# apache/orc

Measured on AMD Instinct MI355X. Metric: decoded GB/s + Mvalues/s device-resident, RLEv2 int64 column at 1/2/4/8 GPU, higher is better.
Workload: dtype int64; 1 GPU; configs[1]: single int64 RLEv2-direct column, 10^8 rows, uncompressed stream resident in HBM, 1 MI355X per stripe; rows_per_gpu=100000000, encoding=RLEv2 DIRECT, W=64 (aligned), 512-value runs, signed (zigzag), stream_bytes=800390626, row_index_stride=10000, parallelism=stripe-sharded x1, kernel=rlev2_tiled_kernel, variant=0

## Files before the change

orc_amd/csrc/orcg_internal.hh:

```
#pragma once

#include <hip/hip_runtime.h>
#include <stdint.h>

#include <algorithm>
#include <string>
#include <vector>

#include "../../include/orcg.h"

namespace orcg {

enum DevErr : uint32_t {
  kErrNone = 0,
  kErrBadRead = 1,
  kErrPatchedPl0 = 2,
  kErrPatchedWidth = 3,
  kErrDeltaLength = 4,
  kErrBadSegment = 5,
  kErrByteBadRead = 6,
  kErrDictIndex = 7,
  kErrV1BadRead = 8,
  kErrDecimalScale = 9,
  kErrHive11Overflow = 10,
// ... 26 lines not shown
  uint64_t lb_cap = 0;
  uint32_t lb_epoch = 0;
  void* d_rtab = nullptr;
  uint64_t rtab_cap = 0;
  void* d_rhdr = nullptr;
  uint64_t rhdr_cap = 0;
  void* h_jobs = nullptr;
  void* d_jobs = nullptr;
  uint64_t jobs_cap = 0, jobs_used = 0;
  uint8_t* arena_h = nullptr;
  uint8_t* arena_d = nullptr;
  uint64_t arena_cap = 0, arena_used = 0;
  std::vector<Ctx*> lanes;
  hipEvent_t ev_fork = nullptr;
  std::vector<hipEvent_t> ev_join;
};

Ctx* ctx_lane(Ctx* base, size_t k);
void warm_rlev2_walk(hipStream_t s);
void warm_rlev2_tiled(hipStream_t s);
void warm_byterle(hipStream_t s);
void warm_columns(hipStream_t s);
void warm_rlev1(hipStream_t s);
void warm_decimal(hipStream_t s);

unsigned side_lanes();

struct RleJob {
  const uint8_t* src;
  uint64_t src_len;
  const uint64_t* segtab;
  const int64_t* trip;
  const int64_t* rows;
  uint64_t nsegs;
  void* dst;
  uint64_t nvalues;
  uint64_t seg_base;
  uint32_t is_signed;
  uint32_t tab_base;
  unsigned long long* err;
  const uint64_t* dcount;
};

struct V1SegDesc {
  const uint8_t* src;
  uint64_t src_len;
  uint64_t seg_start, vi;
  uint64_t seg_end, v_next;
  void* dst;
  uint64_t nvalues;
  unsigned long long* err;
  uint32_t is_signed, pad;
};

int set_error(Ctx* ctx, int status, const std::string& msg);
bool debug_on(const char* topic);
void debug_stale(const char* where);
void* pinned_alloc(size_t bytes, int node = -1);
int current_numa_node();
void pinned_free(void* p);
int hip_check(Ctx* ctx, hipError_t e, const char* what);
int scratch(Ctx* ctx, int slot, size_t bytes, void** out);
int sync_ctx(Ctx* ctx);

int launch_rlev2_decode(Ctx* ctx, const uint8_t* d_src, uint64_t src_len, int is_signed,
                        const uint64_t* d_segtab, uint64_t nsegs, bool positions_mode,
                        uint64_t rows_per_group, uint64_t value_begin, uint64_t nvalues,
                        void* d_dst, int dst_bytes, int java = 0);


constexpr uint32_t kRtHdr = 6;
constexpr uint32_t kSliceMax = 1024;
struct RunTab {
  uint64_t* tab;
  uint32_t* hdr;
  uint32_t spg;
  uint32_t slice;
};
int launch_rlev2_expand(Ctx* ctx, const uint8_t* d_src, uint64_t src_len, int is_signed, uint64_t value_begin,
                        uint64_t nvalues, void* d_dst, int dst_bytes, const uint64_t* d_count, const RleJob* jobs_d,
                        uint32_t njobs, uint64_t nsegs, const RunTab& rt);
void warm_rlev2_expand(hipStream_t s);

constexpr int kMaxRlev2Variant = 9;
bool rlev2_variant_valid(int v);
int launch_rlev2_tiled(Ctx* ctx, const uint8_t* d_src, uint64_t src_len, int is_signed,
                       const uint64_t* d_segtab, uint64_t nsegs, bool positions_mode,
                       uint64_t rows_per_group, uint64_t value_begin, uint64_t nvalues,
                       void* d_dst, int dst_bytes, const uint64_t* d_count = nullptr);

int launch_rlev2_multi(Ctx* ctx, const RleJob* jobs, uint32_t njobs);
bool rlev2_multi_capable(int variant);
int stage_table(Ctx* ctx, const void* src, size_t bytes, const void** out);
inline int stage_rle_jobs(Ctx* ctx, const RleJob* jobs, uint32_t n, const RleJob** out) {
  return stage_table(ctx, jobs, (size_t)n * sizeof(RleJob), (const void**)out);
}

struct MultiLaunch {
  int kind;
  int variant;
  const void* d_jobs;
  uint32_t njobs;
  uint64_t grid;
  uint64_t values;
  uint64_t tab_entries = 0;
  uint32_t spg = 0, slice = 0;
};
int plan_rlev2_multi(Ctx* ctx, const RleJob* jobs, uint32_t njobs, std::vector<MultiLaunch>& out);
struct VarintJob {
  const uint8_t* src;
  uint64_t len;
  int64_t* counts;
  int64_t* base;
  uint64_t* total;
};
struct ScanJob {
  const int64_t* in;
  uint64_t n;
  int64_t* out;
  uint64_t* flags;
  uint64_t* total;
};
int plan_rlev1_multi(Ctx* ctx, const V1SegDesc* segs, uint64_t nsegs, std::vector<MultiLaunch>& out);
int run_multi(Ctx* ctx, const std::vector<MultiLaunch>& launches);

int launch_byterle(Ctx* ctx, const uint8_t* d_src, uint64_t src_len, const uint64_t* d_segtab, uint64_t nsegs,
                   bool boolean, uint64_t begin, uint64_t nout, uint8_t* d_dst, uint64_t* d_ones = nullptr,
                   const uint64_t* d_nout = nullptr);
int launch_rlev1(Ctx* ctx, const uint8_t* d_src, uint64_t src_len, int is_signed, const uint64_t* d_segtab,
                 uint64_t nsegs, uint64_t value_begin, uint64_t nvalues, void* d_dst, int dst_bytes);
int launch_rlev1_multi(Ctx* ctx, const V1SegDesc* segs, uint64_t nsegs);
int launch_rlev1_jobs(Ctx* ctx, const V1SegDesc* d_segs, uint64_t nsegs, int chunk);
int launch_scatter(Ctx* ctx, const void* d_dense, const uint8_t* d_nn, uint64_t n, void* d_out, int width,
                   int fill_mode, int64_t fill);
int launch_dict_offsets(Ctx* ctx, const int64_t* d_lengths, uint64_t dict_size, int64_t* d_offsets,
                        uint64_t* d_summary = nullptr);
int launch_dict_gather(Ctx* ctx, const void* d_idx, int idx_width, const uint8_t* d_nn, uint64_t n,
                       const int64_t* d_offsets, uint64_t dict_size, int64_t* d_start, int64_t* d_len);
constexpr uint32_t kDictLds = 4096;
struct DictJob {
  const int64_t* lengths;
  uint64_t dict_size;
  int64_t* offsets;
  uint64_t* summary;
  const int64_t* idx;
  const uint8_t* nn;
  uint64_t n;
  int64_t* start;
  int64_t* len;
  unsigned long long* err;
  uint64_t tile_base;
};
int launch_dict_multi(Ctx* ctx, const DictJob* jobs, uint32_t njobs);
int plan_dict_multi(Ctx* ctx, const DictJob* jobs, uint32_t njobs, std::vector<MultiLaunch>& out);
int launch_dict_jobs(Ctx* ctx, const DictJob* d_jobs, uint32_t njobs, uint64_t tiles);

int launch_varint_tile_counts(Ctx* ctx, const uint8_t* d_src, uint64_t len, int64_t* d_counts, uint64_t* ntiles);
constexpr uint64_t kVarintTile = 4096;
int launch_varint_decimal(Ctx* ctx, const uint8_t* d_src, uint64_t len, const int64_t* d_tile_base,
                          const int64_t* d_scales, uint64_t nvalues, int32_t scale, int mode, void* d_out,
                          uint8_t* d_keep = nullptr);
struct DecJob {
  const uint8_t* src;
  uint64_t len;
  const int64_t* tile_base;
  const int64_t* scales;
  uint64_t nvalues;
// ... 67 lines not shown
```

orc_amd/csrc/rlev2_tiled.hip:

```cpp
#include <algorithm>
#include <cstring>
#include <type_traits>
#include <vector>

#include "rlev2_device.hh"

namespace orcg {
namespace {
using namespace dev;

#ifdef ORCG_PHASE_PROF
__device__ unsigned long long g_phase[16];
constexpr uint32_t kWgDurMax = 16384;
__device__ unsigned long long g_wgdur[2 * kWgDurMax];
#define PROF_MARK(k)                                                        \
  do {                                                                      \
    if (threadIdx.x == 0) {                                                 \
      const uint64_t now_ = wall_clock64();                                 \
      atomicAdd(&g_phase[k], (unsigned long long)(now_ - prof_last_));      \
      prof_last_ = now_;                                                    \
    }                                                                       \
  } while (0)
#define PROF_DECL uint64_t prof_last_ = wall_clock64()
#else
#define PROF_MARK(k) \
  do {               \
  } while (0)
#define PROF_DECL
#endif

constexpr int kThreads = 256;
constexpr int kWaves = kThreads / kWave;
constexpr uint32_t kMaxRun = 4608;

constexpr uint32_t kSlab = 2048;
constexpr uint32_t kBlk = kSlab / kThreads;
constexpr uint32_t kDenseRuns = kSlab / 2;
constexpr uint32_t kStage = 256;
constexpr uint32_t kShortL = 16;
constexpr uint32_t kVparL = 256;
#ifndef ORCG_VPAR_MIN
#define ORCG_VPAR_MIN 16
#endif
constexpr uint32_t kVparMin = ORCG_VPAR_MIN;
#ifndef ORCG_VPAR_FRAG
#define ORCG_VPAR_FRAG 2
#endif
constexpr uint32_t kVparFrag = ORCG_VPAR_FRAG;
#ifndef ORCG_FLAT_RUNS
#define ORCG_FLAT_RUNS 2
#endif
constexpr uint32_t kNone = 0xffffffffu;
constexpr uint32_t kDpErr = 0x80000000u;
constexpr uint16_t kSink = 0xffffu;
constexpr uint32_t kWalkDone = 0x80000000u;
constexpr uint32_t kToDense = 24, kToSerial = 64;
#ifndef ORCG_TAB_TO_DENSE
#define ORCG_TAB_TO_DENSE 128
#endif
#ifndef ORCG_TAB_TO_SERIAL
#define ORCG_TAB_TO_SERIAL 512
#endif
constexpr uint32_t kTabToDense = ORCG_TAB_TO_DENSE, kTabToSerial = ORCG_TAB_TO_SERIAL;

constexpr int kOptNTStore = 1;
constexpr int kOptNTLoad = 2;
constexpr int kOptReuse = 4;
constexpr int kOptFast = 8;
constexpr int kOptRegFill = 16;
constexpr int kOptT4 = 32;
constexpr int kOptD3 = 64;
constexpr int kOptDirect = 128;
constexpr int kOptPair = 256;
constexpr int kOptUnion = 1024;
constexpr int kOptScan = 4096;
constexpr int kOptPrefetch = 2048;
constexpr int kOptGrpT = 8192;
constexpr int kOptTable = 16384;
constexpr int kOptFlat = 32768;

#ifdef ORCG_DEBUG_COVER
#define ORCG_COVER_ADD(x) atomicAdd(s_cover_ptr(), (uint32_t)(x))
__device__ __forceinline__ uint32_t* s_cover_ptr() {
  __shared__ uint32_t s_cover;
  return &s_cover;
}
#else
#define ORCG_COVER_ADD(x) \
  do {                    \
  } while (0)
#endif

template <int kOpt, typename T>
__device__ __forceinline__ void store1(T* p, uint64_t v) {
  if constexpr ((kOpt & kOptNTStore) != 0) __builtin_nontemporal_store((T)(int64_t)v, p);
  else *p = (T)(int64_t)v;
}

typedef uint64_t u64x2 __attribute__((ext_vector_type(2)));
template <int kOpt>
__device__ __forceinline__ void store2(int64_t* p, uint64_t a, uint64_t b) {
  u64x2 v;
  v.x = a;
  v.y = b;
  if constexpr ((kOpt & kOptNTStore) != 0) __builtin_nontemporal_store(v, (u64x2*)p);
  else *(u64x2*)p = v;
}

__device__ __forceinline__ uint32_t lds_byte(const uint32_t* w, uint32_t o) {
  return (w[o >> 2] >> ((o & 3u) * 8)) & 0xffu;
}

__device__ __forceinline__ u32x3 lds12(const uint32_t* w, uint32_t o) {
  const uint32_t i = o >> 2;
  u32x3 r;
  r.x = w[i];
  r.y = w[i + 1];
  r.z = w[i + 2];
  return r;
}

constexpr uint32_t kHdrLim = 64;

__device__ __forceinline__ uint32_t term4(uint32_t w) {
  const uint32_t m = (~w >> 7) & 0x01010101u;
  return (m * 0x10204080u) >> 28;
}

struct LaneWin {
  uint32_t word = 0, base = 0xffffffffu;
  uint32_t t4 = 0;
  __device__ __forceinline__ void load(const uint32_t* win, uint32_t hoff, uint32_t nwords, int lane) {
    base = hoff & ~3u;
    uint32_t idx = (base >> 2) + (uint32_t)lane;
    if (idx >= nwords) idx = nwords - 1;
    word = win[idx];
    t4 = term4(word);
  }
  __device__ __forceinline__ void cover(const uint32_t* win, uint32_t hoff, uint32_t nwords, int lane) {
    if (base == 0xffffffffu || hoff < base || hoff + kHdrLim > base + 256) load(win, hoff, nwords, lane);
  }
  __device__ __forceinline__ uint32_t byte(uint32_t o) const {
    o -= base;
    return (rdlane(word, o >> 2) >> ((o & 3u) * 8)) & 0xffu;
  }
};

template <int kOpt, typename T>
__device__ __forceinline__ void expand_run(const uint32_t* win, uint32_t nwords, uint32_t hoff, uint64_t v0,
                                           int is_signed, uint64_t value_begin, uint64_t value_end, T* dst,
                                           int lane) {
  LaneWin hw;
  hw.load(win, hoff, nwords, lane);
  Run r;
  if ((hw.byte(hoff) >> 6) == 3) {
    const uint32_t fb = hw.byte(hoff);
    r.kind = 3;
    r.pbs = r.pl = r.cfb = 0;
    r.err = kErrNone;
    r.L = ((fb & 1u) << 8 | hw.byte(hoff + 1)) + 1u;
    const uint32_t fbo = (fb >> 1) & 0x1fu;
    r.W = fbo ? fbs_width(fbo) : 0u;
// ... 191 lines not shown
    for (int it = 0; it < kMaxRunUnroll; ++it) {
      const uint32_t j = it * kWave + lane;
      const uint64_t o = v0 + j;
      if ((uint32_t)it < niter && j < L && o >= value_begin && o < value_end)
        store1<kOpt>(dst + (o - value_begin), r.a + (uint64_t)j * r.b);
    }
    return;
  }
  const uint32_t W = r.W;
  const uint64_t v1 = r.a + r.b;
  const bool neg = (int64_t)r.b < 0;
  uint64_t carry = 0;
  if (W <= 26 && (kOpt & kOptFast) && L == 512 && v0 >= value_begin && v0 + 512 <= value_end) {
    T* out = dst + (v0 - value_begin);
    uint32_t dl[kMaxRunUnroll];
#pragma unroll
    for (int it = 0; it < kMaxRunUnroll; ++it) {
      const uint32_t j = it * kWave + lane;
      const uint32_t k = j >= 2 ? j - 2 : 0u;
      const uint32_t bit = k * W;
      const uint32_t br = d + (bit >> 3);
      dl[it] = (uint32_t)field(lds12(win, br), br, bit & 7u, W);
    }
    if (lane < 2) dl[0] = 0;
#pragma unroll
    for (int it = 0; it < kMaxRunUnroll; ++it) {
      const uint32_t j = it * kWave + lane;
      const uint32_t s32 = wave_scan_u32(dl[it]);
      const uint64_t sum = carry + s32;
      carry += (uint32_t)__builtin_amdgcn_readlane((int)s32, 63);
      const uint64_t v = j == 0 ? r.a : (j == 1 ? v1 : (neg ? v1 - sum : v1 + sum));
      store1<kOpt>(out + j, v);
    }
    return;
  }
  if (W <= 26) {
#pragma unroll 1
    for (uint32_t it = 0; it < niter; ++it) {
      const uint32_t j = it * kWave + lane;
      const int32_t k = (int32_t)j - 2;
      uint32_t dlt = 0;
      if (k >= 0 && j < L) {
        const uint32_t bit = (uint32_t)k * W;
        const uint32_t br = d + (bit >> 3);
        dlt = (uint32_t)field(lds12(win, br), br, bit & 7u, W);
      }
      const uint32_t s32 = wave_scan_u32(dlt);
      const uint64_t sum = carry + s32;
      carry += (uint32_t)__builtin_amdgcn_readlane((int)s32, 63);
      const uint64_t v = j == 0 ? r.a : (j == 1 ? v1 : (neg ? v1 - sum : v1 + sum));
      const uint64_t o = v0 + j;
      if (j < L && o >= value_begin && o < value_end) store1<kOpt>(dst + (o - value_begin), v);
    }
    return;
  }
#pragma unroll 1
  for (uint32_t it = 0; it < niter; ++it) {
    const uint32_t j = it * kWave + lane;
    const int32_t k = (int32_t)j - 2;
    uint64_t dlt = 0;
    if (k >= 0 && j < L) {
      const uint32_t bit = (uint32_t)k * W;
      const uint32_t br = d + (bit >> 3);
      dlt = field(lds12(win, br), br, bit & 7u, W);
    }
    const uint64_t sum = wave_inclusive_scan(dlt) + carry;
    carry = last_lane(sum);
    const uint64_t v = j == 0 ? r.a : (j == 1 ? v1 : (neg ? v1 - sum : v1 + sum));
    const uint64_t o = v0 + j;
    if (j < L && o >= value_begin && o < value_end) store1<kOpt>(dst + (o - value_begin), v);
  }
}

template <int kOpt>
__device__ __forceinline__ void fill(uint32_t* win, __amdgpu_buffer_rsrc_t rs, uint32_t wrel,
                                     uint32_t bytes, int w, int nw, int lane) {
  for (uint32_t off = w * 1024u; off < bytes; off += nw * 1024u)
    __builtin_amdgcn_raw_ptr_buffer_load_lds(rs, (__attribute__((address_space(3))) void*)((char*)win + off),
                                             16, wrel + off + lane * 16, 0, 0,
                                             (kOpt & kOptNTLoad) ? 2 : 0);
}

__device__ __forceinline__ uint32_t flat_probe(__amdgpu_buffer_rsrc_t rs, uint32_t prel, uint32_t lim,
                                               uint32_t kmax, int lane, uint32_t* nb) {
  uint32_t h[4];
#pragma unroll
  for (uint32_t wi = 0; wi < 4; ++wi) {
    const uint32_t B = 2u + 512u * (5u + wi);
    const uint64_t off = (uint64_t)prel + (uint32_t)lane * B;
    uint32_t x = 0;
    if ((uint32_t)lane < kmax && off + B <= lim) {
      const auto q = __builtin_amdgcn_raw_buffer_load_b64(rs, (uint32_t)off & ~3u, 0, 0);
      const uint64_t qq = ((uint64_t)q[1] << 32) | q[0];
      x = (uint32_t)(qq >> (((uint32_t)off & 3u) * 8u)) & 0xffffu;
    }
    h[wi] = x;
  }
  const uint32_t hdr = uni(h[0]);
  if ((hdr & 0xfff9u) != 0xff79u) return 0;
  const uint32_t wi = (hdr >> 1) & 3u;
  const uint32_t mine = wi == 0 ? h[0] : (wi == 1 ? h[1] : (wi == 2 ? h[2] : h[3]));
  const uint64_t differ = ~__ballot(mine == hdr);
  *nb = 5u + wi;
  return differ ? (uint32_t)__builtin_ctzll(differ) : 64u;
}

template <int kOpt, int kRuns, typename T>
__device__ __forceinline__ void flat_expand(__amdgpu_buffer_rsrc_t rs, uint32_t d, uint32_t dstep, uint32_t nb,
                                            int is_signed, T* out, uint32_t ostep, int lane) {
  u32x3 w[kRuns][kMaxRunUnroll];
#pragma unroll
  for (int q = 0; q < kRuns; ++q) {
#pragma unroll
    for (int it = 0; it < kMaxRunUnroll; ++it) {
      const uint32_t rel = d + (uint32_t)q * dstep + (uint32_t)(it * kWave + lane) * nb;
      const auto t = __builtin_amdgcn_raw_buffer_load_b96(rs, rel & ~3u, 0, 2);
      w[q][it].x = t[0];
      w[q][it].y = t[1];
      w[q][it].z = t[2];
    }
  }
#pragma unroll
  for (int q = 0; q < kRuns; ++q) {
#pragma unroll
    for (int it = 0; it < kMaxRunUnroll; ++it) {
      const uint32_t j = (uint32_t)(it * kWave + lane);
      const uint32_t rel = d + (uint32_t)q * dstep + j * nb;
      uint64_t v = field(w[q][it], rel, 0, 8u * nb);
      if (is_signed) v = unzigzag(v);
      store1<kOpt>(out + (uint32_t)q * ostep + j, v);
    }
  }
}

struct WalkResult {
  uint32_t n, stop, dpos, dval, items, shrt;
};

constexpr uint16_t kItemLong = 0x8000;
#ifndef ORCG_ITEM_MAX
#define ORCG_ITEM_MAX 64
#endif
constexpr uint32_t kItemMax = ORCG_ITEM_MAX;

template <bool kT4>
__device__ __forceinline__ void walk_extent(const LaneWin& hw, uint32_t lp, uint32_t avail, int is_signed,
                                            uint32_t* bytes, uint32_t* L, uint32_t* err, uint32_t* rkind) {
  const uint32_t fb = hw.byte(lp), kind = fb >> 6;
  *err = kErrNone;
  *rkind = kind;
  if (kind < 2) {
    const uint32_t L2 = ((fb & 1u) << 8 | hw.byte(lp + 1)) + 1u;
    const uint32_t db = 2u + (fbs_width((fb >> 1) & 0x1fu) * L2 + 7u) / 8u;
    *bytes = kind ? db : 2u + ((fb >> 3) & 7u);
    *L = kind ? L2 : (fb & 7u) + 3u;
    if (*bytes > avail) *err = kErrBadRead;
    return;
  }
  if (kind != 2) {
    if (avail < 2) {
      *err = kErrBadRead;
      *bytes = 0;
      *L = 0;
      return;
    }
    const uint32_t L2 = ((fb & 1u) << 8 | hw.byte(lp + 1)) + 1u;
    const uint32_t code = (fb >> 1) & 0x1fu;
    const uint32_t o = lp + 2u - hw.base, i0 = o >> 2, sh = o & 3u;
    uint32_t t = 0;
    if constexpr (kT4) {
#pragma unroll
      for (uint32_t k = 0; k < 7; ++k) t |= rdlane(hw.t4, i0 + k) << (4 * k);
      t = (t >> sh) & 0xffffffu;
    } else {
      uint32_t prev = rdlane(hw.word, i0);
#pragma unroll
      for (uint32_t k = 0; k < 6; ++k) {
        const uint32_t nx = rdlane(hw.word, i0 + k + 1);
        t |= term4(__builtin_amdgcn_alignbyte(nx, prev, sh)) << (4 * k);
        prev = nx;
      }
    }
    const uint32_t n1 = t ? (uint32_t)__builtin_ctz(t) + 1u : 32u;
    const uint32_t t2 = n1 < 24 ? t >> n1 : 0u;
    const uint32_t n2 = t2 ? (uint32_t)__builtin_ctz(t2) + 1u : 32u;
    if (n1 <= 11 && n2 <= 11) {
      const uint32_t W = code ? fbs_width(code) : 0u;
      *L = L2;
      if (2u + n1 + n2 > avail) {
        *err = kErrBadRead;
        return;
      }
      if (W != 0 && L2 < 2) {
        *err = kErrDeltaLength;
        return;
      }
      *bytes = 2u + n1 + n2 + (W ? (W * (L2 - 2u) + 7u) / 8u : 0u);
      if (*bytes > avail) *err = kErrBadRead;
      return;
    }
  }
  const Run r = parse_run([&](uint32_t i) { return hw.byte(lp + i); }, avail, kHdrLim, is_signed);
  *bytes = r.bytes;
  *L = r.L;
  *err = r.err;
}

template <uint32_t kWin, uint32_t kCap, bool kT4 = false, typename OffT = uint32_t>
__device__ __forceinline__ WalkResult walk(const uint32_t* win, OffT* run_off, uint32_t* run_val,
                                           uint64_t wpos, uint64_t pos, uint64_t vi, uint64_t seg_end,
                                           uint64_t src_len, uint64_t value_end, int is_signed,
                                           unsigned long long* err, int lane, uint32_t lim = kWin,
                                           uint32_t cap = kCap, uint32_t* pub = nullptr,
// ... 784 lines not shown
    const RleJob* J = jobs + lo;
    src = (const uint8_t*)uni64((uint64_t)(uintptr_t)J->src);
    src_len = uni64(J->src_len);
    is_signed = (int)uni(J->is_signed);
    segtab = (const uint64_t*)uni64((uint64_t)(uintptr_t)J->segtab);
    trip = (const int64_t*)uni64((uint64_t)(uintptr_t)J->trip);
    rows = (const int64_t*)uni64((uint64_t)(uintptr_t)J->rows);
    nsegs = uni64(J->nsegs);
    value_begin = 0;
    const uint64_t jdc = uni64((uint64_t)(uintptr_t)J->dcount);
    value_end = jdc ? uni64(*(const uint64_t*)(uintptr_t)jdc) : uni64(J->nvalues);
    dst = (T*)uni64((uint64_t)(uintptr_t)J->dst);
    const uint64_t je = uni64((uint64_t)(uintptr_t)J->err);
    err = je ? (unsigned long long*)(uintptr_t)je : p_err;
    tab_base = uni(J->tab_base);
    job_idx = lo;
    return gg - uni64(J->seg_base);
  };

  auto run_segment = [&](const uint64_t gg, const bool queued, const uint64_t q_pos, const uint64_t q_vi) {
  const uint64_t g = bind(gg);
  auto seg_at = [&](const uint64_t s, uint64_t* off) -> uint64_t {
    if (kMulti && trip) {
      const int64_t v = rows[s] - trip[3 * s + 1];
      *off = (uint64_t)trip[3 * s];
      return v < 0 ? 0ull : (uint64_t)v;
    }
    *off = segtab[2 * s];
    return kPositions ? s * rows_per_group - segtab[2 * s + 1] : segtab[2 * s + 1];
  };
  uint64_t seg_first = 0;
  const uint64_t vi0 = queued ? 0ull : seg_at(g, &seg_first);
  const uint64_t seg_start = queued ? q_pos : seg_first;
  uint64_t vi = queued ? q_vi : vi0;
  uint64_t seg_end = src_len;
  uint64_t v_next = ~0ull;
  if (g + 1 < nsegs) v_next = seg_at(g + 1, &seg_end);
  if (seg_end > src_len) seg_end = src_len;
  constexpr bool kTable = (kOpt & kOptTable) != 0;
  uint32_t* thdr = nullptr;
  uint64_t* ttab = nullptr;
  uint32_t tcnt = 0;
  const uint64_t tlim = (uint64_t)rtab.spg * rtab.slice;
  if constexpr (kTable) {
    thdr = rtab.hdr + gg * (kRtHdr + rtab.spg);
    const uint32_t tb = tab_base + (uint32_t)(seg_first >> 1) + (uint32_t)g;
    ttab = rtab.tab + tb;
    if (tid == 0) {
      thdr[0] = 0;
      thdr[1] = 0;
      thdr[2] = (uint32_t)vi0;
      thdr[3] = (uint32_t)(vi0 >> 32);
      thdr[4] = tb;
      thdr[5] = job_idx;
    }
  }
  if (vi >= value_end || v_next <= value_begin) return;
  if (seg_start >= seg_end) {
    if (tid == 0 && v_next != ~0ull && v_next != vi && seg_start < src_len) report(err, vi, kErrBadSegment);
    if (tid == 0 && v_next == ~0ull) report(err, vi, kErrBadRead);
    return;
  }

  const uintptr_t base_abs = ((uintptr_t)src + seg_start) & ~(uintptr_t)15;
  const uintptr_t end_abs = ((uintptr_t)src + src_len + 3) & ~(uintptr_t)3;
  const uint64_t span = (uint64_t)(end_abs - base_abs);
  const uint32_t nrec = span > 0xfffff000ull ? 0xfffff000u : (uint32_t)span;
  const __amdgpu_buffer_rsrc_t rs =
      __builtin_amdgcn_make_buffer_rsrc((void*)base_abs, (short)0, (int)nrec, 0x00020000);
  const uint64_t bias = (uint64_t)(base_abs - (uintptr_t)src);

  uint64_t pos = seg_start;
  uint32_t sync_par = 0;
  if (tid < 4) s_sync[tid >> 1][tid & 1] = 0;
  PROF_DECL;
  if constexpr ((kOpt & kOptFlat) != 0 && sizeof(T) == 8 && !kPipe && kDense == 0 && kDefer == 0) {
    if (!queued) {
      const uint64_t flat_end = seg_end < bias + nrec - 4u ? seg_end : bias + nrec - 4u;
      const uint64_t vstop = v_next < value_end ? v_next : value_end;
      const uint32_t wv = uni((uint32_t)wave);
      constexpr int kRuns = ORCG_FLAT_RUNS;
      static_assert(kRuns == 1 || kRuns == 2, "flat runs in flight");
      uint32_t flat_runs = 0;
      while (vi >= value_begin && vi < vstop && pos < flat_end) {
        const uint64_t kv = (vstop - vi) / 512u;
        uint32_t nb = 0;
        const uint32_t m = flat_probe(rs, (uint32_t)(pos - bias), (uint32_t)(flat_end - bias),
                                      kv < 64u ? (uint32_t)kv : 64u, lane, &nb);
        if (m == 0) break;
        const uint32_t B = 2u + 512u * nb;
        const uint32_t d0 = (uint32_t)(pos - bias) + 2u;
        T* const out = dst + (vi - value_begin);
        for (uint32_t r = wv; r < m; r += kWaves * kRuns) {
          if constexpr (kRuns == 2) {
            if (r + kWaves < m) {
              flat_expand<kOpt, 2>(rs, d0 + r * B, kWaves * B, nb, is_signed, out + 512u * r, kWaves * 512u, lane);
              continue;
            }
          }
          flat_expand<kOpt, 1>(rs, d0 + r * B, 0, nb, is_signed, out + 512u * r, 0, lane);
        }
        pos += (uint64_t)m * B;
        vi += 512ull * m;
        flat_runs += m;
        if (m < 64u) break;
      }
      PROF_MARK(7);
#ifdef ORCG_PHASE_PROF
      if (tid == 0) atomicAdd(&g_phase[10], (unsigned long long)flat_runs);
#else
      (void)flat_runs;
#endif
    }
  }
  if constexpr (!kPipe) {
    uint64_t pwpos = ~0ull;
    uint32_t pneed = 0;
    constexpr bool kPf = (kOpt & kOptPrefetch) != 0 && (kOpt & kOptRegFill) != 0 && (kOpt & kOptReuse) != 0 &&
                         kDense == 0;
    typedef uint32_t pf_u4 __attribute__((ext_vector_type(4)));
    constexpr int kPfPer = kPf ? (int)((kWinS + kThreads * 16 - 1) / (kThreads * 16)) : 1;
    pf_u4 pf[kPfPer];
    uint32_t pf_wrel = ~0u, pf_need = 0;
    bool dense = queued;
    bool probe = !queued;
    if constexpr (kDense == 2 && (kOpt & kOptD3) != 0) {
      dense = false;
      probe = true;
    }
    while (pos < seg_end && vi < value_end) {
      const uint32_t wrel = (uint32_t)(pos - bias) & ~15u;
      const uint64_t wpos = bias + wrel;
      const bool big = kUnion && !dense && !probe;
      uint32_t need = big ? kWinS : kWin, keep = 0;
      if constexpr ((kOpt & kOptReuse) != 0) {
        const uint64_t end_rel = (seg_end - bias + 15) & ~15ull;
        if (end_rel - wrel < need) need = (uint32_t)(end_rel - wrel);
        const bool prefetched = kPf && pf_wrel == wrel && pf_need == need;
        if (!prefetched && pwpos != ~0ull && pwpos + pneed > wpos && wpos - pwpos >= pwpos + pneed - wpos) {
          keep = (uint32_t)(pwpos + pneed - wpos);
          if (keep > need) keep = need;
          const uint32_t so = (uint32_t)(wpos - pwpos);
          typedef uint32_t u4 __attribute__((ext_vector_type(4)));
          for (uint32_t o = tid * 16u; o < keep; o += kThreads * 16u)
            *(u4*)((char*)s_win[0] + o) = *(const u4*)((const char*)s_win[0] + so + o);
          __syncthreads();
        }
        if constexpr ((kOpt & kOptRegFill) != 0) {
          typedef uint32_t u4 __attribute__((ext_vector_type(4)));
          constexpr int kPer = (kWinS + kThreads * 16 - 1) / (kThreads * 16);
          if (kPf && prefetched) {
#pragma unroll
            for (int i = 0; i < kPfPer; ++i) {
              const uint32_t off = (uint32_t)(i * kThreads + tid) * 16u;
              if (off < need) *(u4*)((char*)s_win[0] + off) = __builtin_bit_cast(u4, pf[i]);
            }
          } else {
            u4 v[kPer];
#pragma unroll
            for (int i = 0; i < kPer; ++i) {
              const uint32_t off = keep + (uint32_t)(i * kThreads + tid) * 16u;
              if (off < need)
                v[i] = __builtin_bit_cast(u4, __builtin_amdgcn_raw_buffer_load_b128(rs, wrel + off, 0, 2));
            }
#pragma unroll
            for (int i = 0; i < kPer; ++i) {
              const uint32_t off = keep + (uint32_t)(i * kThreads + tid) * 16u;
              if (off < need) *(u4*)((char*)s_win[0] + off) = v[i];
            }
          }
          pf_wrel = ~0u;
        } else {
          for (uint32_t off = keep + wave * 1024u; off < need; off += kWaves * 1024u)
            if (off + lane * 16u < need)
              __builtin_amdgcn_raw_ptr_buffer_load_lds(
                  rs, (__attribute__((address_space(3))) void*)((char*)s_win[0] + off), 16,
// ... 213 lines not shown
        }
        if constexpr (kDense) {
          if (n > 0) {
            const uint32_t bpr = dpos / n;
            if (shrt || (!dense && (n >= 8 || (was_probe && n >= 4)) && bpr < kDenseB)) dense = true;
            else if (dense && bpr >= kSerialB) dense = false;
          }
        }
        if (n == 0 && dpos == 0) break;
        if (big && dense) break;
      } while (pos < wpos + (big ? kChunkS : kChunk) && pos < seg_end && vi < value_end);
      pwpos = wpos;
      pneed = need;
    }
  } else {
    if (wave == 0) {
      const uint32_t wrel = (uint32_t)(pos - bias) & ~15u;
      fill<kOpt>(s_win[0], rs, wrel, kWin, 0, 1, lane);
      asm volatile("s_waitcnt vmcnt(0)" ::: "memory");
      const WalkResult w = walk<kWin, kCap>(s_win[0], s_off[0], s_val[0], bias + wrel, pos, vi, seg_end, src_len,
                                      value_end, is_signed, err, lane);
      if (lane == 0) {
        s_ctl[0][0] = w.n;
        s_ctl[0][1] = w.stop;
        s_ctl[0][2] = w.dpos;
        s_ctl[0][3] = w.dval;
      }
    }
    lds_barrier();
    for (uint32_t b = 0;; b ^= 1) {
      const uint32_t n = uni(s_ctl[b][0]), stop = uni(s_ctl[b][1]);
      const uint64_t next_pos = pos + uni(s_ctl[b][2]), next_vi = vi + uni(s_ctl[b][3]);
      const bool more = !stop && next_pos < seg_end && next_vi < value_end;
      if (wave == 0) {
        if (more) {
          const uint32_t wrel = (uint32_t)(next_pos - bias) & ~15u;
          fill<kOpt>(s_win[b ^ 1], rs, wrel, kWin, 0, 1, lane);
          asm volatile("s_waitcnt vmcnt(0)" ::: "memory");
          const WalkResult w = walk<kWin, kCap>(s_win[b ^ 1], s_off[b ^ 1], s_val[b ^ 1], bias + wrel, next_pos,
                                          next_vi, seg_end, src_len, value_end, is_signed, err, lane);
          if (lane == 0) {
            s_ctl[b ^ 1][0] = w.n;
            s_ctl[b ^ 1][1] = w.stop;
            s_ctl[b ^ 1][2] = w.dpos;
            s_ctl[b ^ 1][3] = w.dval;
          }
        }
      } else {
        for (uint32_t k = wave - 1; k < n; k += kWaves - 1)
          expand_run<kOpt>(s_win[b], kWin / 4 + 8, uni(s_off[b][k]), vi + uni(s_val[b][k]), is_signed, value_begin,
                           value_end, dst, lane);
      }
      lds_barrier();
      if (stop) return;
      pos = next_pos;
      vi = next_vi;
      if (!more) break;
    }
  }
  if (tid == 0 && v_next != ~0ull && vi < value_end && vi != v_next) report(err, vi, kErrBadSegment);
  if (tid == 0 && v_next == ~0ull && vi < value_end) report(err, vi, kErrBadRead);
  };

  if constexpr (kDefer == 2) {
    if (uni64(__hip_atomic_load(&defer_q[3 * p_nsegs], __ATOMIC_RELAXED, __HIP_MEMORY_SCOPE_AGENT)) !=
        (unsigned long long)defer_par)
      return;
    const uint64_t q = blockIdx.x;
    if (q >= p_nsegs || uni64(defer_q[3 * q]) != (unsigned long long)defer_par) return;
    run_segment(q, true, uni64(defer_q[3 * q + 1]), uni64(defer_q[3 * q + 2]));
  } else {
    run_segment(blockIdx.x, false, 0, 0);
  }
#ifdef ORCG_PHASE_PROF
  if (kUnion && tid == 0 && blockIdx.x < kWgDurMax) {
    g_wgdur[2 * blockIdx.x] = wall_clock64() - wg_t0;
    g_wgdur[2 * blockIdx.x + 1] = wg_dense | ((uint64_t)wg_serial << 32);
  }
#endif
}

}

bool rlev2_variant_valid(int v) { return v >= 0 && v <= 9; }

static int defer_queue(Ctx* ctx, uint64_t nsegs, unsigned long long** out) {
  if (ctx->defer_cap < nsegs + 1) {
    if (ctx->d_defer) {
      (void)hipStreamSynchronize(ctx->stream);
      (void)hipFree(ctx->d_defer);
      ctx->d_defer = nullptr;
      ctx->defer_cap = 0;
    }
    const uint64_t cap = std::max<uint64_t>(nsegs + nsegs / 4, 4096);
    int rc = hip_check(ctx, hipMalloc(&ctx->d_defer, 3 * cap * 8), "hipMalloc defer queue");
    if (!rc) rc = hip_check(ctx, hipMemsetAsync(ctx->d_defer, 0, 3 * cap * 8, ctx->stream), "defer queue reset");
    if (rc) return rc;
    ctx->defer_cap = cap;
  }
  *out = (unsigned long long*)ctx->d_defer;
  return ORCG_OK;
}

static int default_variant(uint64_t src_len, uint64_t est_values) {
  return src_len >= 5 * est_values ? 2 : (4 * src_len >= 5 * est_values ? 3 : 6);
}

static int cu_count(Ctx* ctx) {
  if (ctx->num_cus == 0) {
    int cus = 0;
    if (hipDeviceGetAttribute(&cus, hipDeviceAttributeMultiprocessorCount, ctx->device) != hipSuccess || cus <= 0)
      cus = 256;
    ctx->num_cus = cus;
  }
  return ctx->num_cus;
}

constexpr uint64_t kTwoPassSegsPerCu = 12;
static int union_variant(Ctx* ctx, uint64_t nsegs) {
  return nsegs <= kTwoPassSegsPerCu * (uint64_t)cu_count(ctx) ? 6 : 8;
}

static void debug_defer(Ctx* ctx, const unsigned long long* dq, uint64_t nsegs, uint32_t dpar) {
  if (!debug_on("defer")) return;
  std::vector<unsigned long long> h(3 * nsegs + 1);
  if (hipStreamSynchronize(ctx->stream) != hipSuccess ||
      hipMemcpy(h.data(), dq, h.size() * 8, hipMemcpyDeviceToHost) != hipSuccess)
    return;
  uint64_t q = 0;
  for (uint64_t g = 0; g < nsegs; ++g) q += h[3 * g] == dpar ? 1 : 0;
  fprintf(stderr, "defer: %llu of %llu segments queued (any %d)\n", (unsigned long long)q,
          (unsigned long long)nsegs, h[3 * nsegs] == dpar ? 1 : 0);
}

static void two_pass_shape(uint64_t seg_values, uint32_t* spg, uint32_t* slice) {
  const uint64_t n = std::max<uint64_t>(seg_values, 1);
  const uint64_t smax = kSliceMax;
  const uint64_t k = std::min<uint64_t>((n + smax - 1) / smax, 256);
  uint64_t s = (n + k - 1) / k;
  s = std::min<uint64_t>((s + 255) & ~255ull, smax);
  *spg = (uint32_t)k;
  *slice = (uint32_t)s;
}

static uint64_t seg_value_bound(uint64_t values, uint64_t nsegs) {
  const uint64_t avg = (values + nsegs - 1) / std::max<uint64_t>(nsegs, 1);
  return avg + avg / 8 + 512;
}

static int runtab_buffers(Ctx* ctx, uint64_t entries, uint64_t nsegs, uint32_t spg, uint32_t slice, RunTab* rt) {
  const uint64_t tb = std::max<uint64_t>(entries, 1) * 8, hb = nsegs * (kRtHdr + spg) * 4;
  if (ctx->rtab_cap < tb || ctx->rhdr_cap < hb) {
    (void)hipStreamSynchronize(ctx->stream);
    if (ctx->rtab_cap < tb) {
      if (ctx->d_rtab) (void)hipFree(ctx->d_rtab);
      ctx->d_rtab = nullptr;
      ctx->rtab_cap = 0;
      const uint64_t cap = std::max<uint64_t>(tb + tb / 4, 1u << 20);
      int rc = hip_check(ctx, hipMalloc(&ctx->d_rtab, cap), "hipMalloc run table");
      if (rc) return rc;
      ctx->rtab_cap = cap;
    }
    if (ctx->rhdr_cap < hb) {
      if (ctx->d_rhdr) (void)hipFree(ctx->d_rhdr);
      ctx->d_rhdr = nullptr;
      ctx->rhdr_cap = 0;
      const uint64_t cap = std::max<uint64_t>(hb + hb / 4, 256u << 10);
// ... 18 lines not shown
    if (jobs_d) {
      if (ml && ml->spg) {
        entries = ml->tab_entries;
        spg = ml->spg;
        slice = ml->slice;
      }
    } else if (src_len < 0xffff0000ull && nsegs < 0x7fff0000ull) {
      entries = src_len / 2 + nsegs + 1;
      bound = positions_mode ? rows_per_group + 512 : seg_value_bound(nvalues, nsegs);
      two_pass_shape(bound, &spg, &slice);
    }
    if (spg && entries < 0xffff0000ull && nsegs * spg < 0x7fffffffull) {
      const int rc = runtab_buffers(ctx, entries, nsegs, spg, slice, &rtab);
      if (rc) return rc;
    } else {
      variant = 8;
    }
  }
  if (nsegs > 0x7fffffffull) return set_error(ctx, ORCG_INVALID_ARGUMENT, "too many segments");
  if (dst_bytes != 8 && dst_bytes != 4 && dst_bytes != 2)
    return set_error(ctx, ORCG_INVALID_ARGUMENT, "dst_bytes must be 8, 4 or 2");
  const dim3 block(kThreads);
  const int sg = is_signed ? 1 : 0;
  unsigned long long* dq = nullptr;
  uint32_t dpar = 0;
  (void)cu_count(ctx);

#define ORCG_K(T, P, O, WKB, PIPE, ML)                                                               \
  hipLaunchKernelGGL((rlev2_tiled_kernel<T, P, O, WKB, PIPE, MW, DN, DF, ML>), grid, block, 0, ctx->stream,   \
                     d_src, src_len, sg, d_segtab, nsegs, rows_per_group, value_begin, nvalues, (T*)d_dst, \
                     ctx->d_err, dq, dpar, jobs_d, njobs_d, dcount, rtab)
#define ORCG_KX1(O, WKB, PIPE, MWV, DNV, DFV, GRIDV)                                 \
  do {                                                                              \
    constexpr int MW = MWV;                                                         \
    constexpr int DN = (int)(DNV);                                                  \
    constexpr int DF = DFV;                                                         \
    const dim3 grid(GRIDV);                                                         \
    if (dst_bytes == 8) {                                                           \
      if (positions_mode) ORCG_K(int64_t, true, O, WKB, PIPE, false);                \
      else ORCG_K(int64_t, false, O, WKB, PIPE, false);                              \
    } else if (dst_bytes == 4) {                                                    \
      if (positions_mode) ORCG_K(int32_t, true, O, WKB, PIPE, false);                \
      else ORCG_K(int32_t, false, O, WKB, PIPE, false);                              \
    } else {                                                                        \
      if (positions_mode) ORCG_K(int16_t, true, O, WKB, PIPE, false);                \
      else ORCG_K(int16_t, false, O, WKB, PIPE, false);                              \
    }                                                                               \
  } while (0)
#define ORCG_KX(O, WKB, PIPE, MWV, DNV, DFV, GRIDV)                                  \
  do {                                                                              \
    constexpr int MW = MWV;                                                         \
    constexpr int DN = (int)(DNV);                                                  \
    constexpr int DF = DFV;                                                         \
    const dim3 grid(GRIDV);                                                         \
    if (jobs_d) {                                                                   \
      ORCG_K(int64_t, false, O, WKB, PIPE, true);                                   \
    } else if (dst_bytes == 8) {                                                    \
      if (positions_mode) ORCG_K(int64_t, true, O, WKB, PIPE, false);                \
      else ORCG_K(int64_t, false, O, WKB, PIPE, false);                              \
    } else if (dst_bytes == 4) {                                                    \
      if (positions_mode) ORCG_K(int32_t, true, O, WKB, PIPE, false);                \
      else ORCG_K(int32_t, false, O, WKB, PIPE, false);                              \
    } else {                                                                        \
      if (positions_mode) ORCG_K(int16_t, true, O, WKB, PIPE, false);                \
      else ORCG_K(int16_t, false, O, WKB, PIPE, false);                              \
    }                                                                               \
  } while (0)
#define ORCG_KT(O, WKB, PIPE, MWV, DNV) ORCG_KX1(O, WKB, PIPE, MWV, DNV, 0, grid_s)

  constexpr int kSer = kOptNTStore | kOptReuse | kOptFast | kOptT4;
  constexpr int kWide = kSer | kOptRegFill;
#define ORCG_DEFERRING(O, WKB, MWV, DO)                                               \
  do {                                                                              \
    int rc_ = defer_queue(ctx, nsegs, &dq);                                          \
    if (rc_) return rc_;                                                            \
    dpar = (uint32_t)(ctx->defer_seq++ % 0xffffffffull) + 1u;          \
    ORCG_KX(O, WKB, false, MWV, 0, 1, (unsigned)nsegs);                              \
    debug_defer(ctx, dq, nsegs, dpar);                                                \
    ORCG_KX(DO, 8, false, 6, 2, 2, (unsigned)nsegs);                                 \
  } while (0)

  const unsigned grid_s = (unsigned)nsegs;
  switch (variant) {
    case 2: ORCG_KX(kWide | kOptD3 | kOptFlat, 33, false, 1, 0, 0, grid_s); break;
    case 3: ORCG_DEFERRING(kSer | kOptD3, 21, 6, kSer | kOptD3); break;
    case 4: ORCG_KX(kSer | kOptD3, 8, false, 6, 2, 0, grid_s); break;
    case 5: ORCG_KX(kSer | kOptD3, 12, false, 5, 2, 0, grid_s); break;
    case 6: {
      ORCG_KX(kSer | kOptD3 | kOptUnion | kOptTable, 8, false, 6, 2, 0, grid_s);
      const int rc = hip_check(ctx, hipGetLastError(), "rlev2_tiled_kernel launch");
      if (rc) return rc;
      return launch_rlev2_expand(ctx, d_src, src_len, sg, value_begin, nvalues, d_dst, dst_bytes, dcount, jobs_d,
                                 njobs_d, nsegs, rtab);
    }
    case 7: ORCG_DEFERRING(kWide | kOptD3, 33, 1, kSer | kOptD3); break;
    case 8: ORCG_KX(kSer | kOptD3 | kOptUnion, 8, false, 6, 2, 0, grid_s); break;
    case 9: ORCG_KX(kWide | kOptD3, 33, false, 1, 0, 0, grid_s); break;
    default: return set_error(ctx, ORCG_INVALID_ARGUMENT, "unknown RLEv2 kernel variant");
  }
#undef ORCG_DEFERRING
#undef ORCG_KT
#undef ORCG_KX
#undef ORCG_KX1
#undef ORCG_K
  return hip_check(ctx, hipGetLastError(), "rlev2_tiled_kernel launch");
}

int launch_rlev2_tiled(Ctx* ctx, const uint8_t* d_src, uint64_t src_len, int is_signed,
                       const uint64_t* d_segtab, uint64_t nsegs, bool positions_mode,
                       uint64_t rows_per_group, uint64_t value_begin, uint64_t nvalues, void* d_dst,
                       int dst_bytes, const uint64_t* d_count) {
  int variant = ctx->rlev2_variant;
  if (variant == 0) {
    const uint64_t est = positions_mode ? nsegs * rows_per_group : nvalues;
    variant = default_variant(src_len, est);
    if (variant == 6) variant = union_variant(ctx, nsegs);
    else if (variant == 2 && 10 * src_len > 81 * est) variant = 6;
  }
  return launch_tiled(ctx, variant, d_src, src_len, is_signed, d_segtab, nsegs, positions_mode, rows_per_group,
                      value_begin, nvalues, d_dst, dst_bytes, nullptr, 0, d_count);
}

int stage_table(Ctx* ctx, const void* src, size_t bytes, const void** out) {
  const uint64_t need = (bytes + 255) & ~(uint64_t)255;
  if (ctx->arena_h) {
    if (ctx->arena_used + need > ctx->arena_cap) return set_error(ctx, ORCG_INVALID_ARGUMENT, "job arena full");
    memcpy(ctx->arena_h + ctx->arena_used, src, bytes);
    *out = ctx->arena_d + ctx->arena_used;
    ctx->arena_used += need;
    return ORCG_OK;
  }
  if (ctx->jobs_cap < need) {
    (void)hipStreamSynchronize(ctx->stream);
    if (ctx->d_jobs) (void)hipFree(ctx->d_jobs);
    if (ctx->h_jobs) (void)hipHostFree(ctx->h_jobs);
    ctx->d_jobs = ctx->h_jobs = nullptr;
    ctx->jobs_cap = ctx->jobs_used = 0;
    const uint64_t cap = std::max<uint64_t>(4 * need, 256u << 10);
    int rc = hip_check(ctx, hipMalloc(&ctx->d_jobs, cap), "hipMalloc job table");
    if (!rc) rc = hip_check(ctx, hipHostMalloc(&ctx->h_jobs, cap, hipHostMallocDefault), "hipHostMalloc job table");
    if (rc) return rc;
    ctx->jobs_cap = cap;
  }
  if (ctx->jobs_used + need > ctx->jobs_cap) {
    int rc = hip_check(ctx, hipStreamSynchronize(ctx->stream), "job ring wrap");
    if (rc) return rc;
    ctx->jobs_used = 0;
  }
  uint8_t* h = (uint8_t*)ctx->h_jobs + ctx->jobs_used;
  uint8_t* d = (uint8_t*)ctx->d_jobs + ctx->jobs_used;
  memcpy(h, src, bytes);
  ctx->jobs_used += need;
  *out = d;
  return hip_check(ctx, hipMemcpyAsync(d, h, bytes, hipMemcpyHostToDevice, ctx->stream), "H2D jobs");
}

bool rlev2_multi_capable(int variant) { return variant == 0 || (variant >= 2 && variant <= 9); }

int plan_rlev2_multi(Ctx* ctx, const RleJob* jobs, uint32_t njobs, std::vector<MultiLaunch>& out) {
  const int pinned = ctx->rlev2_variant;
  if (!rlev2_multi_capable(pinned)) {
    for (uint32_t j = 0; j < njobs; ++j) {
      if (!jobs[j].segtab) return set_error(ctx, ORCG_INVALID_ARGUMENT, "row-index job needs a multi-stream instance");
      out.push_back(MultiLaunch{3, pinned, jobs + j, 1, jobs[j].nsegs, jobs[j].nvalues});
    }
    return ORCG_OK;
  }
  std::vector<RleJob> group[10];
  for (uint32_t j = 0; j < njobs; ++j) {
    const RleJob& J = jobs[j];
    if (J.nsegs == 0 || J.nvalues == 0) continue;
    group[pinned ? pinned : default_variant(J.src_len, J.nvalues)].push_back(J);
  }
  if (debug_on("jobs"))
    for (int v = 2; v <= 9; ++v)
      for (const RleJob& J : group[v])
        fprintf(stderr, "rle job: instance %d bytes %llu values %llu segments %llu (%.3f B/value)\n", v,
                (unsigned long long)J.src_len, (unsigned long long)J.nvalues, (unsigned long long)J.nsegs,
                (double)J.src_len / (double)J.nvalues);
  for (int v = 2; v <= 9; ++v) {
    std::vector<RleJob>& g = group[v];
    if (g.empty()) continue;
    std::stable_sort(g.begin(), g.end(), [](const RleJob& a, const RleJob& b) {
      return (double)a.src_len * (double)b.nvalues > (double)b.src_len * (double)a.nvalues;
    });
    uint64_t segs = 0, values = 0, entries = 0, bound = 0;
    for (RleJob& J : g) {
      J.seg_base = segs;
      segs += J.nsegs;
      values += J.nvalues;
      J.tab_base = (uint32_t)std::min<uint64_t>(entries, 0xffffffffull);
      entries += J.src_len / 2 + J.nsegs + 1;
      bound = std::max(bound, seg_value_bound(J.nvalues, J.nsegs));
    }
    if (segs > 0x7fffffffull) return set_error(ctx, ORCG_INVALID_ARGUMENT, "too many segments");
    const RleJob* d = nullptr;
    const int rc = stage_rle_jobs(ctx, g.data(), (uint32_t)g.size(), &d);
    if (rc) return rc;
    const int lv = (v == 6 && !pinned) ? union_variant(ctx, segs) : v;
    MultiLaunch m{0, lv, d, (uint32_t)g.size(), segs, values};
    if (lv == 6 && entries < 0xffff0000ull) {
      m.tab_entries = entries;
      two_pass_shape(bound, &m.spg, &m.slice);
    }
    out.push_back(m);
  }
  return ORCG_OK;
}

int run_multi(Ctx* ctx, const std::vector<MultiLaunch>& ls) {
  int ninst = 0, crit = -1;
  bool aux = false;
  for (size_t i = 0; i < ls.size(); ++i) {
    const MultiLaunch& m = ls[i];
    if (m.kind == 1 || m.kind == 4) aux = true;
    if (m.kind != 0) continue;
    ++ninst;
    const bool two = m.spg > 0, ctwo = crit >= 0 && ls[crit].spg > 0;
    if (crit < 0 || (two && !ctwo) || (two == ctwo && m.values > ls[crit].values)) crit = (int)i;
  }
  const int nlanes = (ninst > 0 ? ninst - 1 : 0) + (aux && ninst > 0 ? 1 : 0);
  const bool par = nlanes > 0 && side_lanes() > 1 && (size_t)nlanes <= side_lanes() &&
                   ctx_lane(ctx, (size_t)nlanes - 1) != nullptr;
  Ctx* const base = ctx;
  int used = 0, aux_lane = -1, rc = ORCG_OK;
  if (par) rc = hip_check(ctx, hipEventRecord(ctx->ev_fork, ctx->stream), "fork event");
  auto fork = [&](Ctx** c) -> int {
    *c = base->lanes[used++];
    return hip_check(base, hipStreamWaitEvent((*c)->stream, base->ev_fork, 0), "fork wait");
  };
  bool joined = false;
  auto join = [&]() -> int {
    int r = ORCG_OK;
    for (int k = 0; k < used; ++k) {
      int jr = hip_check(base, hipEventRecord(base->ev_join[k], base->lanes[k]->stream), "join event");
      if (!jr) jr = hip_check(base, hipStreamWaitEvent(base->stream, base->ev_join[k], 0), "join wait");
      if (jr && !r) r = jr;
    }
    joined = true;
    return r;
  };
  for (size_t i = 0; i < ls.size() && !rc; ++i) {
    const MultiLaunch& m = ls[i];
    if ((m.kind == 2 || m.kind == 5 || m.kind == 6) && !joined && (rc = join())) break;
    debug_stale("run_multi: before a launch");
    if (m.kind == 0) {
      Ctx* c = base;
      if (par && (int)i != crit && (rc = fork(&c))) break;
      unsigned long long* const own = c->d_err;
      c->d_err = base->d_err;
      rc = launch_tiled(c, m.variant, nullptr, 0, 0, nullptr, m.grid, false, 0, 0, m.values, nullptr, 8,
                        (const RleJob*)m.d_jobs, m.njobs, nullptr, &m);
      c->d_err = own;
      if (rc) {
        char b[160];
        snprintf(b, sizeof b, " (instance %d, %u streams, %llu segments%s)", m.variant, m.njobs,
                 (unsigned long long)m.grid, c == base ? "" : ", side lane");
        base->last_error = c->last_error + b;
      }
    } else if (m.kind == 1 || m.kind == 4) {
      Ctx* c = base;
      if (par && !joined) {
        if (aux_lane < 0) {
// ... 72 lines not shown
```

Baseline: 2845 GB/s.

## Add 16-byte vector load path for 64-bit-wide flat RLEv2 direct runs

For flat direct runs with 8-byte width, the new path loads each run's bytes with aligned 128-bit buffer loads and keeps several runs in flight. It reassembles unaligned big-endian values with lane shifts (DPP) and alignbyte, and optionally writes with 16-byte stores. This replaces the per-value unaligned field extraction, aiming for fewer, wider memory transactions. It is enabled in variant 2 (the likely default), keeps the old flat path as variant 10, adds experimental variants behind a macro, and tightens the probe bound for the wide case. The cost is more registers and extra lane-crossing instructions.

```diff
diff --git a/orc_amd/csrc/orcg_internal.hh b/orc_amd/csrc/orcg_internal.hh
--- a/orc_amd/csrc/orcg_internal.hh
+++ b/orc_amd/csrc/orcg_internal.hh
@@ -132,7 +132,11 @@
                         uint32_t njobs, uint64_t nsegs, const RunTab& rt);
 void warm_rlev2_expand(hipStream_t s);
 
-constexpr int kMaxRlev2Variant = 9;
+#ifdef ORCG_FLAT16_STEPS
+constexpr int kMaxRlev2Variant = 14;
+#else
+constexpr int kMaxRlev2Variant = 10;
+#endif
 bool rlev2_variant_valid(int v);
 int launch_rlev2_tiled(Ctx* ctx, const uint8_t* d_src, uint64_t src_len, int is_signed,
                        const uint64_t* d_segtab, uint64_t nsegs, bool positions_mode,
diff --git a/orc_amd/csrc/rlev2_tiled.hip b/orc_amd/csrc/rlev2_tiled.hip
--- a/orc_amd/csrc/rlev2_tiled.hip
+++ b/orc_amd/csrc/rlev2_tiled.hip
@@ -50,6 +50,12 @@
 #ifndef ORCG_FLAT_RUNS
 #define ORCG_FLAT_RUNS 2
 #endif
+#ifndef ORCG_FLAT16_RUNS
+#define ORCG_FLAT16_RUNS 5
+#endif
+#ifndef ORCG_FLAT16_STORE16
+#define ORCG_FLAT16_STORE16 0
+#endif
 constexpr uint32_t kNone = 0xffffffffu;
 constexpr uint32_t kDpErr = 0x80000000u;
 constexpr uint16_t kSink = 0xffffu;
@@ -78,6 +84,9 @@
 constexpr int kOptGrpT = 8192;
 constexpr int kOptTable = 16384;
 constexpr int kOptFlat = 32768;
+constexpr int kOptFlat16 = 65536;
+constexpr int kOptF16Runs2 = 1 << 17, kOptF16Runs3 = 1 << 18, kOptF16Runs5 = 1 << 19, kOptF16St8 = 1 << 20,
+              kOptF16St16 = 1 << 21;
 
 #ifdef ORCG_DEBUG_COVER
 #define ORCG_COVER_ADD(x) atomicAdd(s_cover_ptr(), (uint32_t)(x))
@@ -435,14 +444,14 @@
 }
 
 __device__ __forceinline__ uint32_t flat_probe(__amdgpu_buffer_rsrc_t rs, uint32_t prel, uint32_t lim,
-                                               uint32_t kmax, int lane, uint32_t* nb) {
+                                               uint32_t lim64, uint32_t kmax, int lane, uint32_t* nb) {
   uint32_t h[4];
 #pragma unroll
   for (uint32_t wi = 0; wi < 4; ++wi) {
     const uint32_t B = 2u + 512u * (5u + wi);
     const uint64_t off = (uint64_t)prel + (uint32_t)lane * B;
     uint32_t x = 0;
-    if ((uint32_t)lane < kmax && off + B <= lim) {
+    if ((uint32_t)lane < kmax && off + B <= (wi == 3 ? lim64 : lim)) {
       const auto q = __builtin_amdgcn_raw_buffer_load_b64(rs, (uint32_t)off & ~3u, 0, 0);
       const uint64_t qq = ((uint64_t)q[1] << 32) | q[0];
       x = (uint32_t)(qq >> (((uint32_t)off & 3u) * 8u)) & 0xffffu;
@@ -482,6 +491,76 @@
       uint64_t v = field(w[q][it], rel, 0, 8u * nb);
       if (is_signed) v = unzigzag(v);
       store1<kOpt>(out + (uint32_t)q * ostep + j, v);
+    }
+  }
+}
+
+typedef uint32_t u32x4 __attribute__((ext_vector_type(4)));
+
+__device__ __forceinline__ uint32_t next_lane(uint32_t x, uint32_t last) {
+  return (uint32_t)__builtin_amdgcn_update_dpp((int)last, (int)x, 0x130, 0xf, 0xf, false);
+}
+
+template <int kOpt, int K>
+__device__ __forceinline__ void flat16_run(const u32x4 (&c)[4], uint32_t e, int e0, uint32_t r, int is_signed,
+                                           bool st16, int64_t* out, int lane) {
+#pragma unroll
+  for (int it = 0; it < 4; ++it) {
+    uint32_t D[8];
+#pragma unroll
+    for (int k = 0; k < 4; ++k) D[k] = c[it][k];
+#pragma unroll
+    for (int k = 0; k <= K; ++k) D[4 + k] = next_lane(c[it][k], it < 3 ? uni(c[it < 3 ? it + 1 : 3][k]) : rdlane(e, e0 + k));
+    uint64_t v[2];
+#pragma unroll
+    for (int h = 0; h < 2; ++h) {
+      const uint32_t lo = __builtin_amdgcn_alignbyte(D[K + 2 * h + 1], D[K + 2 * h], r);
+      const uint32_t hi = __builtin_amdgcn_alignbyte(D[K + 2 * h + 2], D[K + 2 * h + 1], r);
+      v[h] = ((uint64_t)__builtin_bswap32(lo) << 32) | __builtin_bswap32(hi);
+      if (is_signed) v[h] = unzigzag(v[h]);
+    }
+    int64_t* const o = (int64_t*)((char*)out + 16u * (uint32_t)lane) + 2 * kWave * it;
+    if (st16) {
+      store2<kOpt>(o, v[0], v[1]);
+    } else {
+      store1<kOpt>(o, v[0]);
+      store1<kOpt>(o + 1, v[1]);
+    }
+  }
+}
+
+template <int kOpt, int kRuns, bool kSt16>
+__device__ __forceinline__ void flat_expand16(__amdgpu_buffer_rsrc_t rs, uint32_t d, uint32_t dstep, uint32_t cnt,
+                                              int is_signed, int64_t* out, uint32_t ostep, int lane) {
+  cnt = uni(cnt);
+  d = uni(d);
+  u32x4 c[kRuns][4];
+  const uint32_t l16 = 16u * (uint32_t)lane;
+#pragma unroll
+  for (int q = 0; q < kRuns; ++q) {
+    if ((uint32_t)q < cnt) {
+      const uint32_t a = (d + (uint32_t)q * dstep) & ~15u;
+#pragma unroll
+      for (int it = 0; it < 4; ++it)
+        c[q][it] = __builtin_amdgcn_raw_buffer_load_b128(rs, l16, a + 1024u * (uint32_t)it, 2);
+    }
+  }
+  static_assert(4 * kRuns <= kWave, "one lane per dword of the runs' last chunks");
+  const uint32_t eq = (uint32_t)lane >> 2 < cnt ? (uint32_t)lane >> 2 : cnt - 1u;
+  const uint32_t e =
+      __builtin_amdgcn_raw_buffer_load_b32(rs, ((d + eq * dstep) & ~15u) + 4096u + 4u * ((uint32_t)lane & 3u), 0, 2);
+  const bool st16 = kSt16 && uni((uint32_t)(uintptr_t)out & 15u) == 0;
+#pragma unroll
+  for (int q = 0; q < kRuns; ++q) {
+    if ((uint32_t)q < cnt) {
+      const uint32_t s = (d + (uint32_t)q * dstep) & 15u;
+      int64_t* const o = out + (uint32_t)q * ostep;
+      switch (s >> 2) {
+        case 0: flat16_run<kOpt, 0>(c[q], e, 4 * q, s & 3u, is_signed, st16, o, lane); break;
+        case 1: flat16_run<kOpt, 1>(c[q], e, 4 * q, s & 3u, is_signed, st16, o, lane); break;
+        case 2: flat16_run<kOpt, 2>(c[q], e, 4 * q, s & 3u, is_signed, st16, o, lane); break;
+        default: flat16_run<kOpt, 3>(c[q], e, 4 * q, s & 3u, is_signed, st16, o, lane); break;
+      }
     }
   }
 }
@@ -1432,16 +1511,37 @@
       constexpr int kRuns = ORCG_FLAT_RUNS;
       static_assert(kRuns == 1 || kRuns == 2, "flat runs in flight");
       uint32_t flat_runs = 0;
+      constexpr bool kF16 = (kOpt & kOptFlat16) != 0;
+      constexpr int kRuns16 = (kOpt & kOptF16Runs2) ? 2 : (kOpt & kOptF16Runs3) ? 3 : (kOpt & kOptF16Runs5) ? 5
+                                                                                                        : ORCG_FLAT16_RUNS;
+      static_assert(kRuns16 == 2 || kRuns16 == 3 || kRuns16 == 5, "flat 16-byte runs in flight");
+      constexpr bool kSt16 = (kOpt & kOptF16St16) != 0 || (ORCG_FLAT16_STORE16 != 0 && (kOpt & kOptF16St8) == 0);
+      uint32_t lim64 = (uint32_t)(flat_end - bias);
+      if constexpr (kF16) {
+        const uint64_t rel_end = seg_end - bias;
+        lim64 = nrec < 16u ? 0u : (uint32_t)(rel_end < nrec - 16u ? rel_end : nrec - 16u);
+      }
       while (vi >= value_begin && vi < vstop && pos < flat_end) {
         const uint64_t kv = (vstop - vi) / 512u;
         uint32_t nb = 0;
-        const uint32_t m = flat_probe(rs, (uint32_t)(pos - bias), (uint32_t)(flat_end - bias),
+        const uint32_t m = flat_probe(rs, (uint32_t)(pos - bias), (uint32_t)(flat_end - bias), lim64,
                                       kv < 64u ? (uint32_t)kv : 64u, lane, &nb);
         if (m == 0) break;
         const uint32_t B = 2u + 512u * nb;
         const uint32_t d0 = (uint32_t)(pos - bias) + 2u;
         T* const out = dst + (vi - value_begin);
-        for (uint32_t r = wv; r < m; r += kWaves * kRuns) {
+        bool wide16 = false;
+        if constexpr (kF16) {
+          if (nb == 8u) {
+            wide16 = true;
+            for (uint32_t r = wv; r < m; r += kWaves * kRuns16) {
+              const uint32_t left = (m - r + kWaves - 1) / kWaves;
+              flat_expand16<kOpt, kRuns16, kSt16>(rs, d0 + r * B, kWaves * B, left < (uint32_t)kRuns16 ? left : kRuns16,
+                                                  is_signed, (int64_t*)out + 512u * r, kWaves * 512u, lane);
+            }
+          }
+        }
+        for (uint32_t r = wv; !wide16 && r < m; r += kWaves * kRuns) {
           if constexpr (kRuns == 2) {
             if (r + kWaves < m) {
               flat_expand<kOpt, 2>(rs, d0 + r * B, kWaves * B, nb, is_signed, out + 512u * r, kWaves * 512u, lane);
@@ -1821,7 +1921,7 @@
 
 }
 
-bool rlev2_variant_valid(int v) { return v >= 0 && v <= 9; }
+bool rlev2_variant_valid(int v) { return v >= 0 && v <= kMaxRlev2Variant; }
 
 static int defer_queue(Ctx* ctx, uint64_t nsegs, unsigned long long** out) {
   if (ctx->defer_cap < nsegs + 1) {
@@ -2006,7 +2106,9 @@
 
   const unsigned grid_s = (unsigned)nsegs;
   switch (variant) {
-    case 2: ORCG_KX(kWide | kOptD3 | kOptFlat, 33, false, 1, 0, 0, grid_s); break;
+    case 2:
+      ORCG_KX(kWide | kOptD3 | kOptFlat | kOptFlat16, 33, false, 1, 0, 0, grid_s);
+      break;
     case 3: ORCG_DEFERRING(kSer | kOptD3, 21, 6, kSer | kOptD3); break;
     case 4: ORCG_KX(kSer | kOptD3, 8, false, 6, 2, 0, grid_s); break;
     case 5: ORCG_KX(kSer | kOptD3, 12, false, 5, 2, 0, grid_s); break;
@@ -2020,6 +2122,13 @@
     case 7: ORCG_DEFERRING(kWide | kOptD3, 33, 1, kSer | kOptD3); break;
     case 8: ORCG_KX(kSer | kOptD3 | kOptUnion, 8, false, 6, 2, 0, grid_s); break;
     case 9: ORCG_KX(kWide | kOptD3, 33, false, 1, 0, 0, grid_s); break;
+    case 10: ORCG_KX(kWide | kOptD3 | kOptFlat, 33, false, 1, 0, 0, grid_s); break;
+#ifdef ORCG_FLAT16_STEPS
+    case 11: ORCG_KX1(kWide | kOptD3 | kOptFlat | kOptFlat16 | kOptF16Runs2 | kOptF16St8, 33, false, 1, 0, 0, grid_s); break;
+    case 12: ORCG_KX1(kWide | kOptD3 | kOptFlat | kOptFlat16 | kOptF16Runs2 | kOptF16St16, 33, false, 1, 0, 0, grid_s); break;
+    case 13: ORCG_KX1(kWide | kOptD3 | kOptFlat | kOptFlat16 | kOptF16Runs3 | kOptF16St8, 33, false, 1, 0, 0, grid_s); break;
+    case 14: ORCG_KX1(kWide | kOptD3 | kOptFlat | kOptFlat16 | kOptF16Runs5 | kOptF16St8, 33, false, 1, 0, 0, grid_s); break;
+#endif
     default: return set_error(ctx, ORCG_INVALID_ARGUMENT, "unknown RLEv2 kernel variant");
   }
 #undef ORCG_DEFERRING
@@ -2079,7 +2188,7 @@
   return hip_check(ctx, hipMemcpyAsync(d, h, bytes, hipMemcpyHostToDevice, ctx->stream), "H2D jobs");
 }
 
-bool rlev2_multi_capable(int variant) { return variant == 0 || (variant >= 2 && variant <= 9); }
+bool rlev2_multi_capable(int variant) { return variant == 0 || (variant >= 2 && variant <= 10); }
 
 int plan_rlev2_multi(Ctx* ctx, const RleJob* jobs, uint32_t njobs, std::vector<MultiLaunch>& out) {
   const int pinned = ctx->rlev2_variant;
@@ -2090,19 +2199,19 @@
     }
     return ORCG_OK;
   }
-  std::vector<RleJob> group[10];
+  std::vector<RleJob> group[11];
   for (uint32_t j = 0; j < njobs; ++j) {
     const RleJob& J = jobs[j];
     if (J.nsegs == 0 || J.nvalues == 0) continue;
     group[pinned ? pinned : default_variant(J.src_len, J.nvalues)].push_back(J);
   }
   if (debug_on("jobs"))
-    for (int v = 2; v <= 9; ++v)
+    for (int v = 2; v <= 10; ++v)
       for (const RleJob& J : group[v])
         fprintf(stderr, "rle job: instance %d bytes %llu values %llu segments %llu (%.3f B/value)\n", v,
                 (unsigned long long)J.src_len, (unsigned long long)J.nvalues, (unsigned long long)J.nsegs,
                 (double)J.src_len / (double)J.nvalues);
-  for (int v = 2; v <= 9; ++v) {
+  for (int v = 2; v <= 10; ++v) {
     std::vector<RleJob>& g = group[v];
     if (g.empty()) continue;
     std::stable_sort(g.begin(), g.end(), [](const RleJob& a, const RleJob& b) {
```

Result: faster. 2919 GB/s (median of 6 runs) (+2.6%).
